# rgl-epfl/differentiable-sdf-rendering

Hardware: AMD Instinct MI355X
Metric: diff-renders/sec (fwd+bwd) 256^3 SDF, 512^2, 12 views (higher is better)
Workload: dtype f32; 1 GPU; no-tex-12-hq sizes: 256^3 SDF, 12 views x 512^2, sdf_silhouette_reparam, spp primal/grad 256/64 (reference semantics, configs.py:16,19); views_total=12, views_this_rank=12, partition=whole views, spp_primal=256, spp_grad=64, schedule=primal pass and gradient sweep on two HIP streams

## Files before the change

### differentiable-sdf-rendering_amd/csrc/dsdf_kernels.hip

```cpp
#include <hip/hip_runtime.h>
#include <stdio.h>
#include <stdlib.h>
#include <string.h>
#include <mutex>
#include <vector>
#include "dsdf_lane.h"

using namespace dsdf;

#if DSDF_XF
namespace dsdf {
__constant__ XfState g_xf_dev;
XfState g_xf_host = {{1.f, 0.f, 0.f, 0.f, 1.f, 0.f, 0.f, 0.f, 1.f}, {0.f, 0.f, 0.f}, {0.f, 0.f, 0.f}, {1.f, 1.f, 1.f}};
}
#endif

#define DSDF_BLOCK 256
#define DSDF_TSTRIDE 68
#define DSDF_TROWS 13
#define DSDF_WAVE_LDS 1104
#ifndef DSDF_PRIMAL_MINWAVES
#define DSDF_PRIMAL_MINWAVES 8
#endif

// ... 770 lines not shown
    uint32_t *count0;
    unsigned char *skip;
    uint32_t *items;
    char *tail;
    size_t tail_bytes;
    float *hit_t;
    char *shq;
    uint32_t shq_cap_sub;
    uint32_t cap, nunits, tail_cap_sub, tail_words, group_views, coef_rows;
    size_t bytes;
};

static Workspace carve(void *base, int W, int H, int spp, int nv, int integrator, bool diff = true) {
    Workspace ws;
    const size_t nch = (size_t)film_channels(integrator), rows = integrator == DSDF_DIRECT ? 27 : 9;
    size_t Wb = W + 2 * DSDF_BORDER, Hb = H + 2 * DSDF_BORDER;
    size_t nunits;
    int tile_w, tile_h;
    pass_shape(W, H, spp, tile_w, tile_h, nunits);
    size_t cap = nunits * 64;
    size_t off = 0;
    char *p = (char *)base;
    ws.block = (float *)(p + off); off += align_up(nv * Wb * Hb * nch * sizeof(float), 256);
    ws.skip = (unsigned char *)(p + off); off += align_up(nv * Wb * Hb, 256);
    ws.items = (uint32_t *)(p + off); off += align_up((DSDF_MAX_GROUPS * DSDF_ITEM_HDR + nv * Wb * Hb) * sizeof(uint32_t), 256);
    ws.block_adj = nullptr; ws.count = nullptr; ws.qlane = nullptr; ws.qrec = nullptr; ws.qcoef = nullptr; ws.coef_rows = 0; ws.count0 = nullptr;
    ws.tail = nullptr; ws.tail_bytes = 0; ws.tail_cap_sub = 0; ws.tail_words = 0; ws.hit_t = nullptr; ws.shq = nullptr; ws.shq_cap_sub = 0;
    ws.group_views = (uint32_t)((nv + DSDF_MAX_GROUPS - 1) / DSDF_MAX_GROUPS);
    if (diff) {
        ws.block_adj = (float *)(p + off); off += align_up(nv * Wb * Hb * nch * sizeof(float), 256);
        ws.count = (uint32_t *)(p + off); off += align_up(nv * nunits * sizeof(uint32_t), 256);
        ws.qlane = (uint32_t *)(p + off); off += align_up(nv * cap * sizeof(uint32_t), 256);
        ws.qrec = (float *)(p + off); off += align_up(nv * cap * rows * sizeof(float), 256);
        if (integrator != DSDF_DIRECT) {
            ws.coef_rows = integrator == DSDF_SILHOUETTE ? 8 : DSDF_COEF_WORDS;
            ws.qcoef = (float *)(p + off); off += align_up(nv * cap * ws.coef_rows * sizeof(float), 256);
            ws.count0 = (uint32_t *)(p + off); off += align_up(nv * nunits * sizeof(uint32_t), 256);
        }
    }
    if (spp % 64 == 0) {
        const size_t handoff = diff ? DSDF_TAIL_HANDOFF : DSDF_PTAIL_HANDOFF;
        ws.tail_words = diff ? DSDF_TAIL_WORDS : DSDF_PTAIL_WORDS;
        ws.tail_cap_sub = (uint32_t)((ws.group_views * Wb * Hb * (size_t)(spp / 64) + DSDF_TAIL_SUBQ - 1) / DSDF_TAIL_SUBQ * handoff);
        ws.tail_bytes = align_up((size_t)DSDF_MAX_GROUPS * DSDF_TAIL_SUBQ * DSDF_TAIL_CNT_STRIDE * sizeof(uint32_t), 256) +
                        (size_t)DSDF_MAX_GROUPS * align_up((size_t)DSDF_TAIL_SUBQ * ws.tail_cap_sub * ws.tail_words * sizeof(float), 256);
        ws.tail = p + off; off += ws.tail_bytes;
    }
// ... 189 lines not shown
    hipLaunchKernelGGL(k_pad_grid, dim3(grid), dim3(256), 0, (hipStream_t)stream, data, rx, ry, rz, padded);
    int rc = check_launch("k_pad_grid");
    if (rc) return rc;
    float *c0 = padded + n;
    for (int l = 0; l < DSDF_COARSE_LEVELS; ++l) {
        int cx, cy, cz;
        coarse_dims(rx, ry, rz, l, cx, cy, cz);
        int nc = cx * cy * cz;
        float *c1 = c0 + nc;
        hipLaunchKernelGGL(k_coarse_reduce<false>, dim3((nc + 63) / 64), dim3(64), 0, (hipStream_t)stream, data, rx, ry, rz, c0, cx, cy, cz,
                           1 << DSDF_COARSE_SHIFT(l));
        hipLaunchKernelGGL(k_coarse_dilate<false>, dim3((nc + 63) / 64), dim3(64), 0, (hipStream_t)stream, c0, c1, cx, cy, cz, 1);
        c0 = c1 + nc;
    }
    {
        int cx, cy, cz;
        hit_dims(rx, ry, rz, cx, cy, cz);
        int nc = cx * cy * cz;
        float *c1 = c0 + nc;
        hipLaunchKernelGGL(k_coarse_reduce<true>, dim3((nc + 255) / 256), dim3(256), 0, (hipStream_t)stream, data, rx, ry, rz, c0, cx, cy, cz,
                           1 << DSDF_HIT_SHIFT);
        hipLaunchKernelGGL(k_coarse_dilate<true>, dim3((nc + 255) / 256), dim3(256), 0, (hipStream_t)stream, c0, c1, cx, cy, cz, DSDF_HIT_RADIUS);
    }
    {
        float *F = fine_buffer(padded, rx, ry, rz), *S = F + (size_t)rx * ry * rz;
        const size_t total = (size_t)rx * ry * rz;
        const dim3 g((unsigned)((total + 255) / 256)), b(256);
        const hipStream_t st = (hipStream_t)stream;
#if DSDF_TLAYOUT
        float *T = padded + tlayout_offset(rx, ry, rz);
        hipLaunchKernelGGL(k_window<false>, g, b, 0, st, data, S, total, rx, (size_t)1, DSDF_FINE_LO, DSDF_FINE_HI);
        hipLaunchKernelGGL(k_window<false>, g, b, 0, st, (const float *)S, T, total, ry, (size_t)rx, DSDF_FINE_LO, DSDF_FINE_HI);
        hipLaunchKernelGGL(k_window<false>, g, b, 0, st, (const float *)T, S, total, rz, (size_t)rx * ry, DSDF_FINE_LO, DSDF_FINE_HI);
#else
        float *T = S;
#endif
        hipLaunchKernelGGL(k_window<true>, g, b, 0, st, data, F, total, rx, (size_t)1, DSDF_FINE_LO, DSDF_FINE_HI);
        hipLaunchKernelGGL(k_window<true>, g, b, 0, st, (const float *)F, T, total, ry, (size_t)rx, DSDF_FINE_LO, DSDF_FINE_HI);
        hipLaunchKernelGGL(k_window<true>, g, b, 0, st, (const float *)T, F, total, rz, (size_t)rx * ry, DSDF_FINE_LO, DSDF_FINE_HI);
    }
    if ((rc = check_launch("k_coarse_reduce/dilate/window"))) return rc;
#if DSDF_TLAYOUT
    {
        const int sx = rx + 2 * DSDF_APRON, sy = ry + 2 * DSDF_APRON, sz = rz + 2 * DSDF_APRON, nxc = (int)tlayout_chunks(rx);
        const size_t nt = (size_t)nxc * sz * sy * 2;
        const int tg = (int)((nt + 255) / 256 < 16384 ? (nt + 255) / 256 : 16384);
// ... 128 lines not shown
    return g_events[g_next_event++ % g_events.size()];
}

static thread_local unsigned long long *g_tail_stats = nullptr;
static thread_local hipEvent_t g_time_ev[2] = {nullptr, nullptr};
static thread_local int g_time_state = 0;

static void timing_mark(int which, hipStream_t st) {
    if (g_time_state != 1 && !(which == 1 && g_time_state == 3)) return;
    if (which == 0) { if (hipEventRecord(g_time_ev[0], st) == hipSuccess) g_time_state = 3; }
    else { if (hipEventRecord(g_time_ev[1], st) == hipSuccess) g_time_state = 2; }
}

struct SkipShare {
    unsigned char *buf = nullptr;
    size_t bytes = 0;
    bool valid = false;
    hipEvent_t ready = nullptr;
    int device = -1;
    const float *padded = nullptr;
    int rx = 0, ry = 0, rz = 0, W = 0, H = 0, nv = 0;
    int hit_proof = 0;
    int fine_empty = 0;
    dsdf_params prm;
    dsdf_camera cams[DSDF_MAX_BATCH];
};
static thread_local SkipShare t_share;

static bool skip_share_matches(const SkipShare &h, const PassCtx &c, const dsdf_camera *cams, int nv) {
    return h.valid && h.padded == c.padded && h.rx == c.rx && h.ry == c.ry && h.rz == c.rz && h.W == c.W && h.H == c.H && h.nv == nv &&
           h.hit_proof <= (int)(c.integrator == DSDF_SILHOUETTE && !(c.flags & DSDF_NO_HIT_PROOF)) &&
           h.fine_empty <= (int)!(c.flags & DSDF_NO_FINE_EMPTY) &&
           memcmp(&h.prm, c.prm, sizeof(dsdf_params)) == 0 && memcmp(h.cams, cams, (size_t)nv * sizeof(dsdf_camera)) == 0;
}

static int pixel_proof(const PassCtx &c, const Workspace &ws, const dsdf_camera *cams, int nv, const ViewBatch &VB,
                       const unsigned char *&skip) {
    int rc;
    hipStream_t st = c.st;
    const size_t npix = c.Wb * c.Hb;
    skip = nullptr;
    float step = 0.f;
    const int level = (c.flags & DSDF_NO_SKIP) ? -1 : skip_level(cams, nv, c.W, c.rx, c.ry, c.rz, step);
    if (level < 0) return DSDF_OK;
    SkipShare &sh = t_share;
    const bool can_share = sh.buf && sh.ready && sh.bytes >= (size_t)nv * npix;
    if (can_share && skip_share_matches(sh, c, cams, nv)) {
        if (hipStreamWaitEvent(st, sh.ready, 0) != hipSuccess) return fail(DSDF_ERR_LAUNCH, "hipStreamWaitEvent(shared skip flags) failed");
        skip = sh.buf;
        return DSDF_OK;
    }
    unsigned char *dst = (can_share && !sh.valid) ? sh.buf : ws.skip;
    const bool want_hit = c.integrator == DSDF_SILHOUETTE && !(c.flags & DSDF_NO_HIT_PROOF) && c.spp >= HIT_PROOF_MIN_SPP;
    const float hstep = want_hit ? hit_step(cams, nv, c.W, c.rx, c.ry, c.rz) : 0.f;
    const float fstep = hit_step_fine(cams, nv, c.W, c.rx, c.ry, c.rz);
    const BoundGrid none = {nullptr, 0, 0, 0, 0, 0.f};
    const BoundGrid fmin = (c.flags & DSDF_NO_FINE_EMPTY) ? none : fine_min_bounds(c.padded, c.rx, c.ry, c.rz);
    const bool fine = fstep > 0.f && (want_hit || fmin.b);
    const int list_g = (fmin.b && (c.diff || dst == sh.buf)) ? 1 : 0;
    uint32_t *und = fine ? ws.items + (size_t)DSDF_MAX_GROUPS * DSDF_ITEM_HDR - DSDF_UNDECIDED_HDR : nullptr;
    if (und && hipMemsetAsync(und, 0, sizeof(uint32_t), st) != hipSuccess) return fail(DSDF_ERR_LAUNCH, "hipMemsetAsync(undecided list) failed");
    const float step0 = level > 0 ? skip_step(cams, nv, c.W, c.rx, c.ry, c.rz, level - 1) : 0.f;
    const dim3 pgrid((unsigned)((npix + 255) / 256), nv), blk(256);
    if ((rc = launch("k_pixel_skip", k_pixel_skip, pgrid, blk, st, device_view(c), min_bounds(c.padded, c.rx, c.ry, c.rz, level > 0 ? level - 1 : 0),
                     min_bounds(c.padded, c.rx, c.ry, c.rz, level), max_bounds(c.padded, c.rx, c.ry, c.rz), c.pp, VB, dst, step0, step, hstep, und, list_g)))
        return rc;
    if (und && (rc = launch("k_pixel_hit_fine", k_pixel_hit_fine, dim3((unsigned)((npix * nv + 255) / 256)), blk, st, device_view(c),
                            fmin, fine_bounds(c.padded, c.rx, c.ry, c.rz), c.pp, VB, dst, und, und + DSDF_UNDECIDED_HDR, fstep, (int)want_hit)))
        return rc;
    if ((rc = launch("k_skip_dilate", k_skip_dilate, pgrid, blk, st, VB, dst))) return rc;
    if (dst == sh.buf) {
        if (hipEventRecord(sh.ready, st) != hipSuccess) return fail(DSDF_ERR_LAUNCH, "hipEventRecord(shared skip flags) failed");
        sh.valid = true; sh.padded = c.padded; sh.rx = c.rx; sh.ry = c.ry; sh.rz = c.rz; sh.W = c.W; sh.H = c.H; sh.nv = nv;
        sh.hit_proof = (int)want_hit;
        sh.fine_empty = (int)(fine && fmin.b);
        sh.prm = *c.prm;
        memcpy(sh.cams, cams, (size_t)nv * sizeof(dsdf_camera));
    }
    skip = dst;
    return DSDF_OK;
}

struct Batch {
    const ViewBatch &VB;
    int nv;
    GridView G;
    ShadeArgs S;
    Queue q;
    float *film;
    const unsigned char *skip;
    unsigned long long *st64;
    bool deep_skip;
    bool env_fill;
};

template <bool DIFF>
static int prefill_film(const PassCtx &c, const Batch &b) {
    int rc;
    const dim3 grid((unsigned)((c.Wb * c.Hb + 255) / 256), b.nv), blk(256);
    if (b.deep_skip && (rc = launch("k_film_ones", k_film_ones, grid, blk, c.st, b.VB, b.skip, b.film, c.row0, c.row1, b.st64))) return rc;
    if (b.env_fill && (rc = launch("k_film_env", k_film_env, grid, blk, c.st, b.VB, b.skip, b.film, c.row0, c.row1,
                                   DIFF ? DSDF_PX_EMPTY_G : (DSDF_PX_EMPTY | DSDF_PX_EMPTY_FINE), b.S.env[0], b.S.env[1], b.S.env[2])))
// ... 448 lines not shown
```

### differentiable-sdf-rendering_amd/csrc/dsdf_proof.h

```cpp
#pragma once
#include "dsdf_math.h"

#define DSDF_PX_EMPTY 1u
#define DSDF_PX_EMPTY_G 2u
#define DSDF_PX_FAR 4u
#define DSDF_PX_FAR_G 8u
#define DSDF_PX_HIT 16u
#define DSDF_PX_DEEP 32u
#define DSDF_PX_ONE 64u
#define DSDF_PX_EMPTY_FINE 128u
#define DSDF_PX_KEEP (DSDF_PX_EMPTY | DSDF_PX_EMPTY_G | DSDF_PX_HIT | DSDF_PX_EMPTY_FINE)

namespace dsdf {

DSDF_HD bool px_primal_empty(unsigned f) { return (f & (DSDF_PX_EMPTY | DSDF_PX_EMPTY_FINE)) != 0u; }
template <bool DIFF> DSDF_HD bool px_skip_trace(unsigned f) { return DIFF ? (f & DSDF_PX_EMPTY_G) != 0u : px_primal_empty(f); }

struct BoundGrid {
    const float *b;
    int cx, cy, cz, shift;
    float off;
};

DSDF_HD float bound_at(const BoundGrid &B, const GridView &G, V3 x) {
// ... 37 lines not shown
    float J = -INFINITY, Jrun = 0.f;
    bool in_run = false;
    for (float tb = t0; tb < t1 + step; tb += 4.f * step) {
        float tc[4], U[4];
#pragma unroll
        for (int k = 0; k < 4; ++k) {
            tc[k] = fminf(tb + (float)k * step, t1);
            U[k] = bound_at(B, G, fma3(tc[k], d, o));
        }
#pragma unroll
        for (int k = 0; k < 4; ++k) {
            if (!(tb + (float)k * step < t1 + step)) break;
            const bool neg = U[k] < 0.f && tc[k] - half >= i0 && tc[k] + half <= i1;
            if (neg) {
                if (!in_run) { in_run = true; Jrun = J; }
                if (tc[k] + half >= Jrun + 1e-4f) return DSDF_PX_HIT;
            } else in_run = false;
            J = fmaxf(J, tc[k] + half + U[k]);
        }
    }
    return 0u;
}

}

static void coarse_dims(int rx, int ry, int rz, int level, int &cx, int &cy, int &cz) {
    const int C = 1 << DSDF_COARSE_SHIFT(level);
    cx = (rx + C - 1) / C; cy = (ry + C - 1) / C; cz = (rz + C - 1) / C;
}
static size_t coarse_cells(int rx, int ry, int rz, int level) {
    int cx, cy, cz;
    coarse_dims(rx, ry, rz, level, cx, cy, cz);
    return (size_t)cx * cy * cz;
}
#define DSDF_HIT_SHIFT 1
#define DSDF_HIT_RADIUS 2
static void hit_dims(int rx, int ry, int rz, int &cx, int &cy, int &cz) {
    const int C = 1 << DSDF_HIT_SHIFT;
    cx = (rx + C - 1) / C; cy = (ry + C - 1) / C; cz = (rz + C - 1) / C;
}
static size_t hit_cells(int rx, int ry, int rz) {
    int cx, cy, cz;
    hit_dims(rx, ry, rz, cx, cy, cz);
    return (size_t)cx * cy * cz;
}

// ... 18 lines not shown
    return step_vox / (float)rmax;
}

static int skip_level(const dsdf_camera *cams, int nv, int W, int rx, int ry, int rz, float &step) {
    for (int level = DSDF_COARSE_LEVELS - 1; level >= 0; --level) {
        step = skip_step(cams, nv, W, rx, ry, rz, level);
        if (step > 0.f) return level;
    }
    step = 0.f;
    return -1;
}

#define DSDF_FINE_LO (-2)
#define DSDF_FINE_HI 3
static float hit_step_fine(const dsdf_camera *cams, int nv, int W, int rx, int ry, int rz) {
    int rmax = rx > ry ? (rx > rz ? rx : rz) : (ry > rz ? ry : rz);
    int rmin = rx < ry ? (rx < rz ? rx : rz) : (ry < rz ? ry : rz);
    const float worst = pixel_spread_voxels(cams, nv, W, rmax);
    if (worst / (float)rmin > 0.5f * DSDF_PROOF_GROW) return 0.f;
    float step_vox = 2.f * (1.f - worst) - 0.02f;
    if (step_vox < 0.25f) return 0.f;
    if (step_vox > 1.f) step_vox = 1.f;
    return step_vox / (float)rmax;
}

static float hit_step(const dsdf_camera *cams, int nv, int W, int rx, int ry, int rz) {
    int rmax = rx > ry ? (rx > rz ? rx : rz) : (ry > rz ? ry : rz);
    int rmin = rx < ry ? (rx < rz ? rx : rz) : (ry < rz ? ry : rz);
    const float worst = pixel_spread_voxels(cams, nv, W, rmax);
    if (worst / (float)rmin > 0.5f * DSDF_PROOF_GROW) return 0.f;
    const float reach = (float)(DSDF_HIT_RADIUS << DSDF_HIT_SHIFT);
    float step_vox = 2.f * (reach - 2.5f - worst);
    if (step_vox < 1.f) return 0.f;
    if (step_vox > 2.f) step_vox = 2.f;
    return step_vox / (float)rmax;
}
```

### differentiable-sdf-rendering_amd/csrc/dsdf_skip.h

```cpp
#pragma once

template <bool MAX>
__global__ void k_coarse_reduce(const float *__restrict__ data, int rx, int ry, int rz, float *__restrict__ c0, int cx, int cy, int cz,
                                int C) {
    int i = blockIdx.x * blockDim.x + threadIdx.x;
    if (i >= cx * cy * cz) return;
    int bx = i % cx, by = (i / cx) % cy, bz = i / (cx * cy);
    float m = MAX ? -INFINITY : INFINITY;
    for (int z = bz * C; z < min(rz, (bz + 1) * C); ++z)
        for (int y = by * C; y < min(ry, (by + 1) * C); ++y)
            for (int x = bx * C; x < min(rx, (bx + 1) * C); ++x) {
                const float v = data[((size_t)z * ry + y) * rx + x];
                m = MAX ? fmaxf(m, v) : fminf(m, v);
            }
    c0[i] = m;
}

template <bool MAX>
__global__ void k_coarse_dilate(const float *__restrict__ c0, float *__restrict__ c, int cx, int cy, int cz, int radius) {
    int i = blockIdx.x * blockDim.x + threadIdx.x;
    if (i >= cx * cy * cz) return;
    int bx = i % cx, by = (i / cx) % cy, bz = i / (cx * cy);
    float m = MAX ? -INFINITY : INFINITY;
    for (int z = max(bz - radius, 0); z <= min(bz + radius, cz - 1); ++z)
        for (int y = max(by - radius, 0); y <= min(by + radius, cy - 1); ++y)
            for (int x = max(bx - radius, 0); x <= min(bx + radius, cx - 1); ++x) {
                const float v = c0[((size_t)z * cy + y) * cx + x];
                m = MAX ? fmaxf(m, v) : fminf(m, v);
            }
    c[i] = m;
}

template <bool MAX>
__global__ void k_window(const float *__restrict__ in, float *__restrict__ out, size_t total, int n, size_t st, int lo, int hi) {
    const size_t i = (size_t)blockIdx.x * blockDim.x + threadIdx.x;
    if (i >= total) return;
    const int a = (int)((i / st) % (size_t)n);
    float m = MAX ? -INFINITY : INFINITY;
    for (int o = lo; o <= hi; ++o) {
        const int b = min(max(a + o, 0), n - 1);
        const float v = in[i + (size_t)(b - a) * st];
        m = MAX ? fmaxf(m, v) : fminf(m, v);
    }
    out[i] = m;
}

#define DSDF_UNDECIDED_HDR 16
__global__ void k_pixel_skip(GridView G, BoundGrid Bmin0, BoundGrid Bmin, BoundGrid Bmax, dsdf_params P, ViewBatch VB,
                             unsigned char *__restrict__ flags, float step0, float step, float hstep, uint32_t *__restrict__ undecided,
                             int list_g) {
    const ViewArgs &A = VB.v[blockIdx.y];
    const int i = blockIdx.x * blockDim.x + threadIdx.x, npix = A.Wb * A.Hb;
    const bool valid = i < npix;
    unsigned f = DSDF_PX_EMPTY;
    if (valid) {
        int py = i / A.Wb, px = i - py * A.Wb;
        CamRay r = camera_ray(A.cam, P, (float)(px - DSDF_BORDER) + 0.5f, (float)(py - DSDF_BORDER) + 0.5f, A.W, A.H);
        V3 d = r.d * rsqf(dot(r.d, r.d));
        if (step0 > 0.f) f = pixel_empty_proof(G, Bmin0, P, r.o, d, step0);
        else f = 0u;
        if (f != (DSDF_PX_EMPTY | DSDF_PX_EMPTY_G) && step > 0.f) f |= pixel_empty_proof(G, Bmin, P, r.o, d, step);
        if (hstep > 0.f && !(f & DSDF_PX_EMPTY)) f |= pixel_hit_proof(G, Bmax, P, r.o, d, hstep);
        flags[(size_t)blockIdx.y * npix + i] = (unsigned char)f;
    }
    if (undecided) {
        const bool open = valid && (!(f & (DSDF_PX_EMPTY | DSDF_PX_HIT)) || (list_g && (f & 3u) == DSDF_PX_EMPTY));
        const uint64_t m = __ballot(open);
        if (m != 0) {
            const int leader = __builtin_ctzll(m);
            uint32_t base = 0;
            if (lane_id() == leader) base = atomicAdd(undecided, (uint32_t)__popcll(m));
            base = (uint32_t)__builtin_amdgcn_readlane((int)base, leader);
            if (open) undecided[DSDF_UNDECIDED_HDR + base + mask_prefix(m)] = (uint32_t)blockIdx.y * (uint32_t)npix + (uint32_t)i;
        }
    }
}

__global__ __launch_bounds__(256) void k_pixel_hit_fine(GridView G, BoundGrid Bmin, BoundGrid B, dsdf_params P, ViewBatch VB,
                                                        unsigned char *__restrict__ flags, const uint32_t *__restrict__ count,
                                                        const uint32_t *__restrict__ list, float step, int hit) {
    const uint32_t i = blockIdx.x * blockDim.x + threadIdx.x;
    if (i >= *count) return;
    const uint32_t e = list[i], npix = (uint32_t)(VB.v[0].Wb * VB.v[0].Hb), view = e / npix, pix = e - view * npix;
    const ViewArgs &A = VB.v[view];
    const int py = (int)(pix / (uint32_t)A.Wb), px = (int)(pix - (uint32_t)py * (uint32_t)A.Wb);
    const CamRay r = camera_ray(A.cam, P, (float)(px - DSDF_BORDER) + 0.5f, (float)(py - DSDF_BORDER) + 0.5f, A.W, A.H);
    const V3 d = r.d * rsqf(dot(r.d, r.d));
    const unsigned f = flags[e];
    unsigned add = 0u;
    if (Bmin.b) {
        const unsigned m = pixel_empty_proof(G, Bmin, P, r.o, d, step);
        add = ((m & DSDF_PX_EMPTY) ? DSDF_PX_EMPTY_FINE : 0u) | (m & DSDF_PX_EMPTY_G);
    }
    if (hit && !add && !(f & DSDF_PX_EMPTY)) add = pixel_hit_proof(G, B, P, r.o, d, step);
    if (add) flags[e] = (unsigned char)(f | add);
}

#define DSDF_FAR_RADIUS 4
__global__ void k_skip_dilate(ViewBatch VB, unsigned char *__restrict__ flags) {
    const ViewArgs &A = VB.v[blockIdx.y];
    int i = blockIdx.x * blockDim.x + threadIdx.x;
    if (i >= A.Wb * A.Hb) return;
    unsigned char *f = flags + (size_t)blockIdx.y * A.Wb * A.Hb;
    int py = i / A.Wb, px = i - py * A.Wb;
    unsigned m = 3u | DSDF_PX_HIT, near = DSDF_PX_HIT;
    for (int y = max(py - DSDF_FAR_RADIUS, 0); y <= min(py + DSDF_FAR_RADIUS, A.Hb - 1); ++y)
        for (int x = max(px - DSDF_FAR_RADIUS, 0); x <= min(px + DSDF_FAR_RADIUS, A.Wb - 1); ++x) {
            const unsigned v = f[y * A.Wb + x];
            m &= v | (px_primal_empty(v) ? DSDF_PX_EMPTY : 0u);
            if (abs(y - py) <= 2 && abs(x - px) <= 2) near &= v;
        }
    f[i] = (unsigned char)((f[i] & DSDF_PX_KEEP) | ((m & 3u) << 2) | ((m & DSDF_PX_HIT) ? DSDF_PX_DEEP : 0u) | (near ? DSDF_PX_ONE : 0u));
}

__global__ void k_film_env(ViewBatch VB, const unsigned char *__restrict__ flags, float *__restrict__ blocks, int row0, int row1,
                           unsigned pass_mask, float er, float eg, float eb) {
    const ViewArgs &A = VB.v[blockIdx.y];
    const int i = blockIdx.x * blockDim.x + threadIdx.x, npix = A.Wb * A.Hb;
    if (i >= npix) return;
    const int py = i / A.Wb, px = i - py * A.Wb;
    if (py < row0 || py >= row1) return;
    const unsigned char *f = flags + (size_t)blockIdx.y * npix;
    bool m = true;
    for (int y = max(py - 2, 0); y <= min(py + 2, A.Hb - 1); ++y)
        for (int x = max(px - 2, 0); x <= min(px + 2, A.Wb - 1); ++x) m = m && (f[y * A.Wb + x] & pass_mask) != 0u;
    if (!m) return;
    float *b = blocks + ((size_t)blockIdx.y * npix + i) * 4;
    atomicAdd(b, er); atomicAdd(b + 1, eg); atomicAdd(b + 2, eb); atomicAdd(b + 3, 1.f);
}

__global__ void k_film_ones(ViewBatch VB, const unsigned char *__restrict__ flags, float *__restrict__ blocks, int row0, int row1,
                            unsigned long long *stats) {
    const ViewArgs &A = VB.v[blockIdx.y];
    const int i = blockIdx.x * blockDim.x + threadIdx.x, npix = A.Wb * A.Hb;
    const int py = i < npix ? i / A.Wb : -1;
// ... 21 lines not shown
#endif
    return G;
}
static BoundGrid min_bounds(const float *padded, int rx, int ry, int rz, int level) {
    const float *c = padded + padded_floats(rx, ry, rz);
    for (int l = 0; l < level; ++l) c += 2 * coarse_cells(rx, ry, rz, l);
    BoundGrid B;
    coarse_dims(rx, ry, rz, level, B.cx, B.cy, B.cz);
    B.shift = DSDF_COARSE_SHIFT(level);
    B.off = 0.f;
    B.b = c + coarse_cells(rx, ry, rz, level);
    return B;
}
static BoundGrid max_bounds(const float *padded, int rx, int ry, int rz) {
    const float *c = padded + padded_floats(rx, ry, rz);
    for (int l = 0; l < DSDF_COARSE_LEVELS; ++l) c += 2 * coarse_cells(rx, ry, rz, l);
    BoundGrid B;
    hit_dims(rx, ry, rz, B.cx, B.cy, B.cz);
    B.shift = DSDF_HIT_SHIFT;
    B.off = 0.f;
    B.b = c + hit_cells(rx, ry, rz);
    return B;
}
static float *fine_buffer(const float *padded, int rx, int ry, int rz) {
    const float *c = padded + padded_floats(rx, ry, rz);
    for (int l = 0; l < DSDF_COARSE_LEVELS; ++l) c += 2 * coarse_cells(rx, ry, rz, l);
    return const_cast<float *>(c) + 2 * hit_cells(rx, ry, rz);
}
static size_t tlayout_offset(int rx, int ry, int rz) {
    size_t n = padded_floats(rx, ry, rz);
    for (int l = 0; l < DSDF_COARSE_LEVELS; ++l) n += 2 * coarse_cells(rx, ry, rz, l);
    n += 2 * hit_cells(rx, ry, rz) + 2 * (size_t)rx * ry * rz;
    return (n + 3) & ~(size_t)3;
}
static BoundGrid fine_bounds(const float *padded, int rx, int ry, int rz) {
    BoundGrid B;
    B.cx = rx; B.cy = ry; B.cz = rz; B.shift = 0; B.off = 0.5f;
    B.b = fine_buffer(padded, rx, ry, rz);
    return B;
}
static BoundGrid fine_min_bounds(const float *padded, int rx, int ry, int rz) {
    BoundGrid B = fine_bounds(padded, rx, ry, rz);
#if DSDF_TLAYOUT
    B.b += (size_t)rx * ry * rz;
#else
    B.b = nullptr;
// ... 4 lines not shown
```

### differentiable-sdf-rendering_amd/python/dsdf/_lib.py

```python
import ctypes as C
import os

_HERE = os.path.dirname(os.path.abspath(__file__))
LIB_PATH = os.environ.get('DSDF_LIB_PATH') or os.path.normpath(os.path.join(_HERE, '..', '..', 'lib', 'libdsdf.so'))

DSDF_SILHOUETTE = 0
DSDF_SIMPLE_SHADING = 1
DSDF_DIRECT = 2
DSDF_REPARAM = 1
DSDF_NO_SKIP = 2
DSDF_NO_HIT_PROOF = 4
DSDF_NO_FINE_EMPTY = 8


class DsdfCamera(C.Structure):
    _fields_ = [('origin', C.c_float * 3), ('left', C.c_float * 3), ('up', C.c_float * 3),
                ('dir', C.c_float * 3), ('tan_half_fov', C.c_float), ('pad', C.c_float * 3)]


class DsdfParams(C.Structure):
    _fields_ = [('trace_eps', C.c_float), ('extra_thresh', C.c_float), ('sil_weight_offset', C.c_float),
                ('sil_weight_epsilon', C.c_float), ('bbox_delta', C.c_float), ('edge_eps', C.c_float),
                ('clamping_thresh', C.c_float), ('near_clip', C.c_float), ('far_clip', C.c_float),
                ('sdf_p', C.c_float * 3), ('weight_strategy', C.c_int), ('refine_steps', C.c_int),
                ('light_dir', C.c_float * 3), ('normalize_warp_field', C.c_int), ('max_reparam_depth', C.c_int)]


class DsdfShading(C.Structure):
    _fields_ = [('albedo', C.c_void_p), ('ax', C.c_int), ('ay', C.c_int), ('az', C.c_int),
                ('env_radiance', C.c_float * 3), ('hide_emitters', C.c_int), ('emitter_samples', C.c_void_p),
                ('grad_albedo', C.c_void_p), ('use_mis', C.c_int), ('variant', C.c_int), ('bsdf_samples', C.c_void_p),
                ('bsdf', C.c_int), ('roughness', C.c_void_p), ('rax', C.c_int), ('ray', C.c_int), ('raz', C.c_int),
                ('grad_roughness', C.c_void_p), ('bsdf_lobe_samples', C.c_void_p)]


# ... 137 lines not shown
```

### differentiable-sdf-rendering_amd/python/dsdf/parallel.py

```python
import math

import torch


def view_shard(n_views, rank, world):
    if world < 1 or not (0 <= rank < world):
        raise ValueError(f"bad rank/world {rank}/{world}")
    base, extra = divmod(n_views, world)
    start = rank * base + min(rank, extra)
    return list(range(start, start + base + (1 if rank < extra else 0)))


def strided_view_shard(indices, rank, world):
    return list(indices)[rank::world]


def work_partition(n_views, film_rows, world):
    if world < 1 or n_views < 1:
        raise ValueError("bad n_views / world")
    tiles = world // math.gcd(n_views, world)
    edges = [round(k * film_rows / tiles) for k in range(tiles + 1)]
    units = [(v, edges[k], edges[k + 1]) for v in range(n_views) for k in range(tiles)]
    return [units[r::world] for r in range(world)]

# ... 14 lines not shown
    for v in sorted(range(n_views), key=lambda i: (-vc[i], i)):
        g = min((g for g in range(G) if len(groups[g]) < per_group), key=lambda g: (sums[g], g))
        groups[g].append(v); sums[g] += vc[v]
    out = []
    for g in range(G):
        views = sorted(groups[g])
        h = cost[views].sum(0) + 1e-12 * max(vc.sum(), 1.0) / rows
        c = np.concatenate([[0.0], np.cumsum(h)])
        edges = [0]
        for k in range(1, tiles):
            e = int(np.searchsorted(c, c[-1] * k / tiles))
            if e > 0 and abs(c[e - 1] - c[-1] * k / tiles) <= abs(c[e] - c[-1] * k / tiles):
                e -= 1
            e = max(edges[-1] + 1, min(e, rows - (tiles - k)))
            edges.append(e)
        edges.append(rows)
        for k in range(tiles):
            out.append([(v, edges[k], edges[k + 1]) for v in views])
    return out


def row_costs(flags, n_views, Wb, Hb, spp, spp_grad, silhouette=True):
    import torch
    f = flags[:n_views * Wb * Hb].view(n_views, Hb, Wb)
    empty, empty_g, far, far_g, hit, deep = ((f & b) != 0 for b in (1, 2, 4, 8, 16, 32))
    listed_p = ~far & ~(deep if silhouette else torch.zeros_like(deep))
    proven_p = listed_p & (empty | (hit if silhouette else torch.zeros_like(hit)))
    traced_p = listed_p & ~proven_p
    listed_g = ~far_g
    traced_g = listed_g & ~empty_g
    cp, cg = spp / 64.0, spp_grad / 64.0
    c = cp * (5600.0 * traced_p.sum(2, dtype=torch.float64) + 500.0 * proven_p.sum(2, dtype=torch.float64)) + \
        cg * (15000.0 * traced_g.sum(2, dtype=torch.float64) + 500.0 * (listed_g & ~traced_g).sum(2, dtype=torch.float64))
    return c


def rank_windows(units):
    out = {}
    for v, r0, r1 in units:
        out.setdefault((r0, r1), []).append(v)
    return sorted(out.items())


def all_reduce_sum(t, group=None):
    import torch.distributed as dist
    if dist.is_available() and dist.is_initialized() and dist.get_world_size(group) > 1:
        dist.all_reduce(t, op=dist.ReduceOp.SUM, group=group)
    return t
# ... 154 lines not shown
        self.seeds, self.seeds_grad = list(seeds), list(seeds_grad)

    def empty_film(self, n):
        return self.r.new_film(n, self.W, self.H, self.integrator, self.grid.device)

    def film(self, views, rows):
        f = self.empty_film(len(views))
        return self.r.render_film(self.grid, [self.sensors[v] for v in views], self.spp, f, rows,
                                  seeds=[self.seeds[v] for v in views], integrator=self.integrator, **self.kw_film)

    def develop(self, film):
        return self.r.develop(film, self.W, self.H, self.integrator)

    def begin_group(self, views):
        import torch
        dev = self.grid.device
        n = len(views) * (self.W + 4) * (self.H + 4)
        self._group_views = list(views)
        bufs = self.__dict__.setdefault('_flag_bufs', [])
        gi = getattr(self, '_group_i', 0)
        self._group_i = gi + 1
        while len(bufs) <= gi:
            bufs.append(None)
        if bufs[gi] is None or bufs[gi].numel() < n:
            bufs[gi] = torch.empty(n, dtype=torch.uint8, device=dev)
        self._flags = bufs[gi]
        self._share_lib = self.r.share_proof_open(self.grid, self.kw.get('shading'), self._flags)

    def end_group(self):
        self.r.share_proof_close(self.grid, self._share_lib)
        self._flag_views = getattr(self, '_group_views', None)

    def row_costs(self):
        views = getattr(self, '_flag_views', None)
        if not views or getattr(self, '_flags', None) is None:
            return [], None
        from .renderer import DSDF_SILHOUETTE
        sil = self.integrator in (DSDF_SILHOUETTE, 'sdf_silhouette_reparam')
        return list(views), row_costs(self._flags, len(views), self.W + 4, self.H + 4, self.spp, self.spp_grad, sil)

    def begin_sweeps(self):
        import torch
        self._next_ws = 0
        self._group_i = 0
        if self._side is not None:
            self._side.wait_stream(torch.cuda.current_stream(self.grid.device))
            self._in_sweeps = True

    def end_sweeps(self):
# ... 141 lines not shown
```

### differentiable-sdf-rendering_amd/python/dsdf/renderer.py

```python
import contextlib
import ctypes as C

import os

import torch

from . import _lib
from ._lib import (DSDF_DIRECT, DSDF_NO_FINE_EMPTY, DSDF_NO_HIT_PROOF, DSDF_NO_SKIP, DSDF_REPARAM, DSDF_SILHOUETTE, DSDF_SIMPLE_SHADING, DsdfCamera,
                   DsdfShading)

INTEGRATORS = {'sdf_silhouette_reparam': DSDF_SILHOUETTE, 'sdf_simple_shading_reparam': DSDF_SIMPLE_SHADING,
               'sdf_direct_reparam': DSDF_DIRECT,
               DSDF_SILHOUETTE: DSDF_SILHOUETTE, DSDF_SIMPLE_SHADING: DSDF_SIMPLE_SHADING, DSDF_DIRECT: DSDF_DIRECT}

STAT_NAMES = ('lanes', 'bbox_lanes', 'steps', 'hits', 'refine_steps', 'warp_active', 'queue_len', 'wave_steps',
              'tail_steps', 'tail_wave_steps', 'tail_rays')
STAT_SLOTS = 16

_workspaces = {}


def _proof_flags(empty_space_skip):
    if empty_space_skip == 'empty-only':
        return DSDF_NO_HIT_PROOF
    if empty_space_skip == 'coarse-empty':
        return DSDF_NO_FINE_EMPTY
    return 0 if empty_space_skip else DSDF_NO_SKIP

MAX_VIEWS_PER_LAUNCH = 16


def _stream():
    return C.c_void_p(torch.cuda.current_stream().cuda_stream)


def _ptr(t):
    return C.c_void_p(t.data_ptr()) if t is not None else C.c_void_p(0)


def _floats(a):
    return (C.c_float * len(a))(*[float(v) for v in a])


def _as_list(sensors):
    return list(sensors) if isinstance(sensors, (list, tuple)) else [sensors]


def _require_dev(t, name, dtype=torch.float32):
    if not isinstance(t, torch.Tensor) or not t.is_cuda:
# ... 548 lines not shown
        yield
    finally:
        share_proof_close(grid, lib)


def _lease_sweep_workspace(dev):
    ent = _sweep_workspaces.get(dev)
    if ent is None or ent['leased']:
        return None, None
    ent['leased'] = True
    return ent['ws'], ent


def step_begin(grid, sensors, spp, spp_grad, seeds, seeds_grad, integrator=DSDF_SILHOUETTE, reparam=True, shading=None,
               grad_albedo=None, empty_space_skip=True):
    sensors = _as_list(sensors)
    W, H = sensors[0].film_size()
    dev = grid.device
    main = torch.cuda.current_stream(dev)
    side = _side_streams.get(dev)
    if side is None:
        side = _side_streams[dev] = torch.cuda.Stream(dev, priority=-1)
    side.wait_stream(main)
    nflag = len(sensors) * (W + 4) * (H + 4)
    flags = _skip_buffers.get(dev)
    if flags is None or flags.numel() < nflag:
        flags = _skip_buffers[dev] = torch.empty(nflag, dtype=torch.uint8, device=dev)
    share = os.environ.get('DSDF_SHARE_SKIP', '1') != '0'
    with torch.cuda.device(dev), (shared_proof(grid, shading, flags) if share else contextlib.nullcontext()):
        ws, lease = _lease_sweep_workspace(dev)
        with torch.cuda.stream(side):
            sweep = GradSweep(grid, sensors, spp_grad, (0, H + 4), seeds=seeds_grad, integrator=integrator, reparam=reparam,
                              shading=shading, grad_albedo=grad_albedo, workspace=ws, empty_space_skip=empty_space_skip)
            if sweep.ws is not None and sweep.ws is not ws:
                if lease is not None:
                    lease['leased'] = False
                lease = _sweep_workspaces[dev] = {'ws': sweep.ws, 'leased': True}
            film_g = sweep.sweep(new_film(len(sensors), W, H, integrator, dev))
        img = render_forward(grid, sensors, spp, seeds=seeds, integrator=integrator, reparam=reparam, shading=shading,
                             empty_space_skip=empty_space_skip)
    return img, StepHandle(sweep, film_g, main, side, lease)


def step_finish(handle, grad_image, grad_grid, grad_p=None):
    if handle.done:
        sw = handle.sweep
        sw.make_private()
# ... 283 lines not shown
```

### include/dsdf.h

```cpp
#ifndef DSDF_H
#define DSDF_H

#include <stddef.h>
#include <stdint.h>

#ifdef __cplusplus
extern "C" {
#endif

#define DSDF_VERSION 308
#define DSDF_STAT_SLOTS 16

enum dsdf_status {
    DSDF_OK = 0,
    DSDF_ERR_INVALID_ARG = -1,
    DSDF_ERR_WORKSPACE = -2,
    DSDF_ERR_LAUNCH = -3,
    DSDF_ERR_NO_DEVICE = -4
};

enum dsdf_integrator {
    DSDF_SILHOUETTE = 0,
    DSDF_SIMPLE_SHADING = 1,
    DSDF_DIRECT = 2
};

enum dsdf_flags {
    DSDF_REPARAM = 1,
    DSDF_NO_SKIP = 2,
    DSDF_NO_HIT_PROOF = 4,
    DSDF_NO_FINE_EMPTY = 8
};

typedef struct dsdf_camera {
    float origin[3];
    float left[3];
    float up[3];
    float dir[3];
    float tan_half_fov;
    float pad[3];
} dsdf_camera;

typedef struct dsdf_params {
    float trace_eps;
    float extra_thresh;
    float sil_weight_offset;
    float sil_weight_epsilon;
    float bbox_delta;
    float edge_eps;
    float clamping_thresh;
    float near_clip;
    float far_clip;
    float sdf_p[3];
    int   weight_strategy;
// ... 153 lines not shown
```

Baseline: 30.79 renders/s.

## Tighten per-pixel empty/hit proofs with a Lipschitz value bound from grid tap differences

Adds a kernel that computes the maximum neighbouring-voxel difference along each axis of the SDF grid. The fine proof pass uses this as a gradient bound, evaluating the actual SDF value with a Lipschitz margin to tighten the min/max bounds along each ray. This lets more pixels be proven empty or hit and skipped in the primal and gradient passes. The proof results go into a second flag plane, so the skip buffers double in size and the dilate and row-cost logic read that plane. The cost is an extra grid reduction and extra SDF evaluations during proof building.

```diff
diff --git a/differentiable-sdf-rendering_amd/csrc/dsdf_kernels.hip b/differentiable-sdf-rendering_amd/csrc/dsdf_kernels.hip
--- a/differentiable-sdf-rendering_amd/csrc/dsdf_kernels.hip
+++ b/differentiable-sdf-rendering_amd/csrc/dsdf_kernels.hip
@@ -816,7 +816,7 @@
     size_t off = 0;
     char *p = (char *)base;
     ws.block = (float *)(p + off); off += align_up(nv * Wb * Hb * nch * sizeof(float), 256);
-    ws.skip = (unsigned char *)(p + off); off += align_up(nv * Wb * Hb, 256);
+    ws.skip = (unsigned char *)(p + off); off += align_up(2 * nv * Wb * Hb, 256);
     ws.items = (uint32_t *)(p + off); off += align_up((DSDF_MAX_GROUPS * DSDF_ITEM_HDR + nv * Wb * Hb) * sizeof(uint32_t), 256);
     ws.block_adj = nullptr; ws.count = nullptr; ws.qlane = nullptr; ws.qrec = nullptr; ws.qcoef = nullptr; ws.coef_rows = 0; ws.count0 = nullptr;
     ws.tail = nullptr; ws.tail_bytes = 0; ws.tail_cap_sub = 0; ws.tail_words = 0; ws.hit_t = nullptr; ws.shq = nullptr; ws.shq_cap_sub = 0;
@@ -1052,6 +1052,11 @@
                            1 << DSDF_HIT_SHIFT);
         hipLaunchKernelGGL(k_coarse_dilate<true>, dim3((nc + 255) / 256), dim3(256), 0, (hipStream_t)stream, c0, c1, cx, cy, cz, DSDF_HIT_RADIUS);
     }
+    if (float *D = grad_bound(padded, rx, ry, rz)) {
+        if (hipMemsetAsync(D, 0, 3 * sizeof(float), (hipStream_t)stream) != hipSuccess) return fail(DSDF_ERR_LAUNCH, "hipMemsetAsync(gradient bound) failed");
+        const unsigned g = (unsigned)((size_t)ry * rz < 4096 ? (size_t)ry * rz : 4096);
+        hipLaunchKernelGGL(k_tap_diff_max, dim3(g), dim3(256), 0, (hipStream_t)stream, data, rx, ry, rz, (int *)D);
+    }
     {
         float *F = fine_buffer(padded, rx, ry, rz), *S = F + (size_t)rx * ry * rz;
         const size_t total = (size_t)rx * ry * rz;
@@ -1226,6 +1231,7 @@
     int rx = 0, ry = 0, rz = 0, W = 0, H = 0, nv = 0;
     int hit_proof = 0;
     int fine_empty = 0;
+    int value_bound = 0;
     dsdf_params prm;
     dsdf_camera cams[DSDF_MAX_BATCH];
 };
@@ -1235,6 +1241,7 @@
     return h.valid && h.padded == c.padded && h.rx == c.rx && h.ry == c.ry && h.rz == c.rz && h.W == c.W && h.H == c.H && h.nv == nv &&
            h.hit_proof <= (int)(c.integrator == DSDF_SILHOUETTE && !(c.flags & DSDF_NO_HIT_PROOF)) &&
            h.fine_empty <= (int)!(c.flags & DSDF_NO_FINE_EMPTY) &&
+           h.value_bound <= (int)!(c.flags & (DSDF_NO_FINE_EMPTY | DSDF_NO_VALUE_BOUND)) &&
            memcmp(&h.prm, c.prm, sizeof(dsdf_params)) == 0 && memcmp(h.cams, cams, (size_t)nv * sizeof(dsdf_camera)) == 0;
 }
 
@@ -1251,7 +1258,7 @@
     const bool can_share = sh.buf && sh.ready && sh.bytes >= (size_t)nv * npix;
     if (can_share && skip_share_matches(sh, c, cams, nv)) {
         if (hipStreamWaitEvent(st, sh.ready, 0) != hipSuccess) return fail(DSDF_ERR_LAUNCH, "hipStreamWaitEvent(shared skip flags) failed");
-        skip = sh.buf;
+        skip = sh.value_bound ? sh.buf + (size_t)nv * npix : sh.buf;
         return DSDF_OK;
     }
     unsigned char *dst = (can_share && !sh.valid) ? sh.buf : ws.skip;
@@ -1262,26 +1269,33 @@
     const BoundGrid fmin = (c.flags & DSDF_NO_FINE_EMPTY) ? none : fine_min_bounds(c.padded, c.rx, c.ry, c.rz);
     const bool fine = fstep > 0.f && (want_hit || fmin.b);
     const int list_g = (fmin.b && (c.diff || dst == sh.buf)) ? 1 : 0;
+    ValueBound vb = {nullptr, 0.f};
+    if (fine && fmin.b && !(c.flags & DSDF_NO_VALUE_BOUND) && (dst != sh.buf || sh.bytes >= 2 * (size_t)nv * npix)) {
+        vb.D = grad_bound(c.padded, c.rx, c.ry, c.rz);
+        vb.r = value_bound_reach(cams, nv, c.W, c.rx, c.ry, c.rz, fstep);
+    }
+    unsigned char *plane = vb.D ? dst + (size_t)nv * npix : nullptr;
     uint32_t *und = fine ? ws.items + (size_t)DSDF_MAX_GROUPS * DSDF_ITEM_HDR - DSDF_UNDECIDED_HDR : nullptr;
     if (und && hipMemsetAsync(und, 0, sizeof(uint32_t), st) != hipSuccess) return fail(DSDF_ERR_LAUNCH, "hipMemsetAsync(undecided list) failed");
     const float step0 = level > 0 ? skip_step(cams, nv, c.W, c.rx, c.ry, c.rz, level - 1) : 0.f;
     const dim3 pgrid((unsigned)((npix + 255) / 256), nv), blk(256);
     if ((rc = launch("k_pixel_skip", k_pixel_skip, pgrid, blk, st, device_view(c), min_bounds(c.padded, c.rx, c.ry, c.rz, level > 0 ? level - 1 : 0),
-                     min_bounds(c.padded, c.rx, c.ry, c.rz, level), max_bounds(c.padded, c.rx, c.ry, c.rz), c.pp, VB, dst, step0, step, hstep, und, list_g)))
+                     min_bounds(c.padded, c.rx, c.ry, c.rz, level), max_bounds(c.padded, c.rx, c.ry, c.rz), c.pp, VB, dst, step0, step, hstep, und, list_g, plane)))
         return rc;
     if (und && (rc = launch("k_pixel_hit_fine", k_pixel_hit_fine, dim3((unsigned)((npix * nv + 255) / 256)), blk, st, device_view(c),
-                            fmin, fine_bounds(c.padded, c.rx, c.ry, c.rz), c.pp, VB, dst, und, und + DSDF_UNDECIDED_HDR, fstep, (int)want_hit)))
+                            fmin, fine_bounds(c.padded, c.rx, c.ry, c.rz), vb, c.pp, VB, dst, plane, und, und + DSDF_UNDECIDED_HDR, fstep, (int)want_hit)))
         return rc;
-    if ((rc = launch("k_skip_dilate", k_skip_dilate, pgrid, blk, st, VB, dst))) return rc;
+    if ((rc = launch("k_skip_dilate", k_skip_dilate, pgrid, blk, st, VB, dst, plane))) return rc;
     if (dst == sh.buf) {
         if (hipEventRecord(sh.ready, st) != hipSuccess) return fail(DSDF_ERR_LAUNCH, "hipEventRecord(shared skip flags) failed");
         sh.valid = true; sh.padded = c.padded; sh.rx = c.rx; sh.ry = c.ry; sh.rz = c.rz; sh.W = c.W; sh.H = c.H; sh.nv = nv;
         sh.hit_proof = (int)want_hit;
         sh.fine_empty = (int)(fine && fmin.b);
+        sh.value_bound = (int)(plane != nullptr);
         sh.prm = *c.prm;
         memcpy(sh.cams, cams, (size_t)nv * sizeof(dsdf_camera));
     }
-    skip = dst;
+    skip = plane ? plane : dst;
     return DSDF_OK;
 }
 
diff --git a/differentiable-sdf-rendering_amd/csrc/dsdf_proof.h b/differentiable-sdf-rendering_amd/csrc/dsdf_proof.h
--- a/differentiable-sdf-rendering_amd/csrc/dsdf_proof.h
+++ b/differentiable-sdf-rendering_amd/csrc/dsdf_proof.h
@@ -83,6 +83,93 @@
     return 0u;
 }
 
+struct ValueBound {
+    const float *D;
+    float r;
+};
+struct ValueMargin { float L, tap; };
+DSDF_HD ValueMargin value_margin(const ValueBound &vb) {
+    const float dn = sqrtf(vb.D[0] * vb.D[0] + vb.D[1] * vb.D[1] + vb.D[2] * vb.D[2]);
+    ValueMargin m;
+    m.L = vb.r * dn * (1.f + 1e-5f);
+    m.tap = 3.f * (vb.D[0] + vb.D[1] + vb.D[2]);
+    return m;
+}
+
+struct HitRun {
+    float J, Jrun;
+    bool in_run, done;
+};
+DSDF_HD void hit_run_step(HitRun &s, float U, float tc, float half, bool inside) {
+    if (s.done) return;
+    if (U < 0.f && inside) {
+        if (!s.in_run) { s.in_run = true; s.Jrun = s.J; }
+        if (tc + half >= s.Jrun + 1e-4f) { s.done = true; return; }
+    } else s.in_run = false;
+    s.J = fmaxf(s.J, tc + half + U);
+}
+
+DSDF_HD unsigned pixel_fine_proofs(const GridView &G, const BoundGrid &Bmin, const BoundGrid &Bmax, const ValueBound &vb, const dsdf_params &P,
+                                   V3 o, V3 d, float step, bool want_hit) {
+    BoxHit b = bbox_ray_intersect(-P.bbox_delta - DSDF_PROOF_GROW, 1.f + P.bbox_delta + DSDF_PROOF_GROW, o, d);
+    if (!(b.hit && b.maxt > 0.f)) return 0u;
+    BoxHit in = bbox_ray_intersect(-P.bbox_delta + DSDF_PROOF_GROW, 1.f + P.bbox_delta - DSDF_PROOF_GROW, o, d);
+    want_hit = want_hit && P.trace_eps > 0.f && in.hit && in.maxt > 0.f;
+    const bool want_empty = Bmin.b != nullptr, third = want_empty && vb.D != nullptr;
+    const float t0 = fmaxf(b.mint, 0.f), t1 = b.maxt, half = 0.5f * step;
+    const float i0 = fmaxf(in.mint, 0.f), i1 = in.maxt;
+    const float thr_p = 2.f * P.trace_eps * fmaxf(t1, 1.f) + 1e-5f;
+    const float thr_g = (P.weight_strategy == 6 ? P.edge_eps * (t1 + 0.1f) : P.edge_eps) * 1.05f + 1e-4f;
+    const float thr_hi = fmaxf(thr_p, thr_g);
+    ValueMargin mg = {0.f, 0.f};
+    if (third) mg = value_margin(vb);
+    float m2 = INFINITY, m3 = INFINITY;
+    HitRun h2 = {-INFINITY, 0.f, false, false}, h3 = h2;
+    bool e_alive = want_empty;
+    for (float tb = t0; tb < t1 + step && (e_alive || (want_hit && !h2.done)); tb += 4.f * step) {
+        float tc[4], lo[4], hi[4], lo3[4], hi3[4];
+        const bool v_alive = third && (e_alive || (want_hit && !h3.done));
+        const bool fetch_lo = e_alive || v_alive;
+#pragma unroll
+        for (int k = 0; k < 4; ++k) {
+            const bool live = tb + (float)k * step < t1 + step;
+            tc[k] = fminf(tb + (float)k * step, t1);
+            const V3 x = fma3(tc[k], d, o);
+            lo3[k] = lo[k] = fetch_lo && live ? bound_at(Bmin, G, x) : INFINITY;
+            hi3[k] = hi[k] = want_hit ? bound_at(Bmax, G, x) : INFINITY;
+            const bool need_e = e_alive && lo[k] <= (m3 > thr_hi ? thr_hi : thr_p);
+            const bool need_h = want_hit && !h3.done && hi[k] >= 0.f && lo[k] < -mg.L;
+            if (v_alive && live && (need_e || need_h)) {
+                const float v = eval_value(G, x), m = mg.L + 4e-6f * (fabsf(v) + mg.tap);
+                lo3[k] = fmaxf(lo[k], v - m);
+                hi3[k] = fminf(hi[k], v + m);
+            }
+        }
+        m2 = fminf(m2, fminf(fminf(lo[0], lo[1]), fminf(lo[2], lo[3])));
+        m3 = fminf(m3, fminf(fminf(lo3[0], lo3[1]), fminf(lo3[2], lo3[3])));
+        if (want_hit) {
+#pragma unroll
+            for (int k = 0; k < 4; ++k) {
+                if (!(tb + (float)k * step < t1 + step)) break;
+                const bool inside = tc[k] - half >= i0 && tc[k] + half <= i1;
+                hit_run_step(h2, hi[k], tc[k], half, inside);
+                hit_run_step(h3, hi3[k], tc[k], half, inside);
+            }
+        }
+        e_alive = want_empty && m3 > thr_p;
+    }
+    unsigned f2 = 0u, f3 = 0u;
+    if (want_empty) {
+        if (m2 > thr_p) f2 |= DSDF_PX_EMPTY;
+        if (m2 > thr_hi) f2 |= DSDF_PX_EMPTY_G;
+        if (m3 > thr_p) f3 |= DSDF_PX_EMPTY;
+        if (m3 > thr_hi) f3 |= DSDF_PX_EMPTY_G;
+    }
+    if (!f2 && want_hit && h2.done) f2 = DSDF_PX_HIT;
+    if (!f3 && want_hit && h3.done) f3 = DSDF_PX_HIT;
+    return third ? (f2 | (f3 << 8)) : f2;
+}
+
 }
 
 static void coarse_dims(int rx, int ry, int rz, int level, int &cx, int &cy, int &cz) {
@@ -147,6 +234,11 @@
     if (step_vox < 0.25f) return 0.f;
     if (step_vox > 1.f) step_vox = 1.f;
     return step_vox / (float)rmax;
+}
+
+static float value_bound_reach(const dsdf_camera *cams, int nv, int W, int rx, int ry, int rz, float fstep) {
+    int rmax = rx > ry ? (rx > rz ? rx : rz) : (ry > rz ? ry : rz);
+    return pixel_spread_voxels(cams, nv, W, rmax) + 0.5f * fstep * (float)rmax + 0.01f;
 }
 
 static float hit_step(const dsdf_camera *cams, int nv, int W, int rx, int ry, int rz) {
diff --git a/differentiable-sdf-rendering_amd/csrc/dsdf_skip.h b/differentiable-sdf-rendering_amd/csrc/dsdf_skip.h
--- a/differentiable-sdf-rendering_amd/csrc/dsdf_skip.h
+++ b/differentiable-sdf-rendering_amd/csrc/dsdf_skip.h
@@ -45,10 +45,32 @@
     out[i] = m;
 }
 
+__global__ __launch_bounds__(256) void k_tap_diff_max(const float *__restrict__ data, int rx, int ry, int rz, int *__restrict__ D) {
+    float mx = 0.f, my = 0.f, mz = 0.f;
+    for (int row = blockIdx.x; row < ry * rz; row += gridDim.x) {
+        const int y = row % ry, z = row / ry;
+        const float *r = data + (size_t)row * rx;
+        for (int x = threadIdx.x; x < rx; x += blockDim.x) {
+            const float v = r[x];
+            if (x + 1 < rx) mx = fmaxf(mx, fabsf(r[x + 1] - v));
+            if (y + 1 < ry) my = fmaxf(my, fabsf(r[x + (size_t)rx] - v));
+            if (z + 1 < rz) mz = fmaxf(mz, fabsf(r[x + (size_t)rx * ry] - v));
+        }
+    }
+    __shared__ int part[4][3];
+    const int ix = wave_max_i32(__float_as_int(mx)), iy = wave_max_i32(__float_as_int(my)), iz = wave_max_i32(__float_as_int(mz));
+    if (lane_id() == 0) { part[threadIdx.x >> 6][0] = ix; part[threadIdx.x >> 6][1] = iy; part[threadIdx.x >> 6][2] = iz; }
+    __syncthreads();
+    if (threadIdx.x < 3) {
+        const int m = max(max(part[0][threadIdx.x], part[1][threadIdx.x]), max(part[2][threadIdx.x], part[3][threadIdx.x]));
+        if (m > __atomic_load_n(D + threadIdx.x, __ATOMIC_RELAXED)) atomicMax(D + threadIdx.x, m);
+    }
+}
+
 #define DSDF_UNDECIDED_HDR 16
 __global__ void k_pixel_skip(GridView G, BoundGrid Bmin0, BoundGrid Bmin, BoundGrid Bmax, dsdf_params P, ViewBatch VB,
                              unsigned char *__restrict__ flags, float step0, float step, float hstep, uint32_t *__restrict__ undecided,
-                             int list_g) {
+                             int list_g, unsigned char *__restrict__ plane) {
     const ViewArgs &A = VB.v[blockIdx.y];
     const int i = blockIdx.x * blockDim.x + threadIdx.x, npix = A.Wb * A.Hb;
     const bool valid = i < npix;
@@ -62,6 +84,7 @@
         if (f != (DSDF_PX_EMPTY | DSDF_PX_EMPTY_G) && step > 0.f) f |= pixel_empty_proof(G, Bmin, P, r.o, d, step);
         if (hstep > 0.f && !(f & DSDF_PX_EMPTY)) f |= pixel_hit_proof(G, Bmax, P, r.o, d, hstep);
         flags[(size_t)blockIdx.y * npix + i] = (unsigned char)f;
+        if (plane) plane[(size_t)blockIdx.y * npix + i] = 0;
     }
     if (undecided) {
         const bool open = valid && (!(f & (DSDF_PX_EMPTY | DSDF_PX_HIT)) || (list_g && (f & 3u) == DSDF_PX_EMPTY));
@@ -76,9 +99,10 @@
     }
 }
 
-__global__ __launch_bounds__(256) void k_pixel_hit_fine(GridView G, BoundGrid Bmin, BoundGrid B, dsdf_params P, ViewBatch VB,
-                                                        unsigned char *__restrict__ flags, const uint32_t *__restrict__ count,
-                                                        const uint32_t *__restrict__ list, float step, int hit) {
+__global__ __launch_bounds__(256) void k_pixel_hit_fine(GridView G, BoundGrid Bmin, BoundGrid B, ValueBound vb, dsdf_params P, ViewBatch VB,
+                                                        unsigned char *__restrict__ flags, unsigned char *__restrict__ plane,
+                                                        const uint32_t *__restrict__ count, const uint32_t *__restrict__ list, float step,
+                                                        int hit) {
     const uint32_t i = blockIdx.x * blockDim.x + threadIdx.x;
     if (i >= *count) return;
     const uint32_t e = list[i], npix = (uint32_t)(VB.v[0].Wb * VB.v[0].Hb), view = e / npix, pix = e - view * npix;
@@ -87,30 +111,37 @@
     const CamRay r = camera_ray(A.cam, P, (float)(px - DSDF_BORDER) + 0.5f, (float)(py - DSDF_BORDER) + 0.5f, A.W, A.H);
     const V3 d = r.d * rsqf(dot(r.d, r.d));
     const unsigned f = flags[e];
-    unsigned add = 0u;
-    if (Bmin.b) {
-        const unsigned m = pixel_empty_proof(G, Bmin, P, r.o, d, step);
-        add = ((m & DSDF_PX_EMPTY) ? DSDF_PX_EMPTY_FINE : 0u) | (m & DSDF_PX_EMPTY_G);
-    }
-    if (hit && !add && !(f & DSDF_PX_EMPTY)) add = pixel_hit_proof(G, B, P, r.o, d, step);
+    const unsigned m = pixel_fine_proofs(G, Bmin, B, vb, P, r.o, d, step, hit && !(f & DSDF_PX_EMPTY));
+    const unsigned m2 = m & 0xffu, m3 = m >> 8;
+    const unsigned add = ((m2 & DSDF_PX_EMPTY) ? DSDF_PX_EMPTY_FINE : 0u) | (m2 & (DSDF_PX_EMPTY_G | DSDF_PX_HIT));
     if (add) flags[e] = (unsigned char)(f | add);
+    const unsigned add3 = ((m3 & DSDF_PX_EMPTY) ? DSDF_PX_EMPTY_FINE : 0u) | (m3 & (DSDF_PX_EMPTY_G | DSDF_PX_HIT));
+    if (plane && add3) plane[e] = (unsigned char)add3;
 }
 
 #define DSDF_FAR_RADIUS 4
-__global__ void k_skip_dilate(ViewBatch VB, unsigned char *__restrict__ flags) {
+__global__ void k_skip_dilate(ViewBatch VB, unsigned char *__restrict__ flags, unsigned char *__restrict__ plane) {
     const ViewArgs &A = VB.v[blockIdx.y];
     int i = blockIdx.x * blockDim.x + threadIdx.x;
     if (i >= A.Wb * A.Hb) return;
     unsigned char *f = flags + (size_t)blockIdx.y * A.Wb * A.Hb;
+    unsigned char *p = plane ? plane + (size_t)blockIdx.y * A.Wb * A.Hb : nullptr;
     int py = i / A.Wb, px = i - py * A.Wb;
-    unsigned m = 3u | DSDF_PX_HIT, near = DSDF_PX_HIT;
+    unsigned m = 3u | DSDF_PX_HIT, near = DSDF_PX_HIT, m3 = m, near3 = near;
     for (int y = max(py - DSDF_FAR_RADIUS, 0); y <= min(py + DSDF_FAR_RADIUS, A.Hb - 1); ++y)
         for (int x = max(px - DSDF_FAR_RADIUS, 0); x <= min(px + DSDF_FAR_RADIUS, A.Wb - 1); ++x) {
             const unsigned v = f[y * A.Wb + x];
             m &= v | (px_primal_empty(v) ? DSDF_PX_EMPTY : 0u);
             if (abs(y - py) <= 2 && abs(x - px) <= 2) near &= v;
+            if (p) {
+                const unsigned w = v | (p[y * A.Wb + x] & DSDF_PX_KEEP);
+                m3 &= w | (px_primal_empty(w) ? DSDF_PX_EMPTY : 0u);
+                if (abs(y - py) <= 2 && abs(x - px) <= 2) near3 &= w;
+            }
         }
-    f[i] = (unsigned char)((f[i] & DSDF_PX_KEEP) | ((m & 3u) << 2) | ((m & DSDF_PX_HIT) ? DSDF_PX_DEEP : 0u) | (near ? DSDF_PX_ONE : 0u));
+    const unsigned own = f[i];
+    f[i] = (unsigned char)((own & DSDF_PX_KEEP) | ((m & 3u) << 2) | ((m & DSDF_PX_HIT) ? DSDF_PX_DEEP : 0u) | (near ? DSDF_PX_ONE : 0u));
+    if (p) p[i] = (unsigned char)(((own | p[i]) & DSDF_PX_KEEP) | ((m3 & 3u) << 2) | ((m3 & DSDF_PX_HIT) ? DSDF_PX_DEEP : 0u) | (near3 ? DSDF_PX_ONE : 0u));
 }
 
 __global__ void k_film_env(ViewBatch VB, const unsigned char *__restrict__ flags, float *__restrict__ blocks, int row0, int row1,
@@ -178,6 +209,12 @@
     B.b = c + hit_cells(rx, ry, rz);
     return B;
 }
+static float *grad_bound(const float *padded, int rx, int ry, int rz) {
+    if (hit_cells(rx, ry, rz) < 3) return nullptr;
+    const float *c = padded + padded_floats(rx, ry, rz);
+    for (int l = 0; l < DSDF_COARSE_LEVELS; ++l) c += 2 * coarse_cells(rx, ry, rz, l);
+    return const_cast<float *>(c);
+}
 static float *fine_buffer(const float *padded, int rx, int ry, int rz) {
     const float *c = padded + padded_floats(rx, ry, rz);
     for (int l = 0; l < DSDF_COARSE_LEVELS; ++l) c += 2 * coarse_cells(rx, ry, rz, l);
diff --git a/differentiable-sdf-rendering_amd/python/dsdf/_lib.py b/differentiable-sdf-rendering_amd/python/dsdf/_lib.py
--- a/differentiable-sdf-rendering_amd/python/dsdf/_lib.py
+++ b/differentiable-sdf-rendering_amd/python/dsdf/_lib.py
@@ -11,6 +11,7 @@
 DSDF_NO_SKIP = 2
 DSDF_NO_HIT_PROOF = 4
 DSDF_NO_FINE_EMPTY = 8
+DSDF_NO_VALUE_BOUND = 16
 
 
 class DsdfCamera(C.Structure):
diff --git a/differentiable-sdf-rendering_amd/python/dsdf/parallel.py b/differentiable-sdf-rendering_amd/python/dsdf/parallel.py
--- a/differentiable-sdf-rendering_amd/python/dsdf/parallel.py
+++ b/differentiable-sdf-rendering_amd/python/dsdf/parallel.py
@@ -60,8 +60,12 @@
 
 def row_costs(flags, n_views, Wb, Hb, spp, spp_grad, silhouette=True):
     import torch
-    f = flags[:n_views * Wb * Hb].view(n_views, Hb, Wb)
-    empty, empty_g, far, far_g, hit, deep = ((f & b) != 0 for b in (1, 2, 4, 8, 16, 32))
+    n = n_views * Wb * Hb
+    f = flags[:n].view(n_views, Hb, Wb)
+    if flags.numel() >= 2 * n:
+        p = flags[n:2 * n].view(n_views, Hb, Wb)
+        f = torch.where(p[0, 0, 0] != 255, p, f)
+    empty, empty_g, far, far_g, hit, deep = ((f & b) != 0 for b in (1 | 128, 2, 4, 8, 16, 32))
     listed_p = ~far & ~(deep if silhouette else torch.zeros_like(deep))
     proven_p = listed_p & (empty | (hit if silhouette else torch.zeros_like(hit)))
     traced_p = listed_p & ~proven_p
@@ -262,9 +266,12 @@
         self._group_i = gi + 1
         while len(bufs) <= gi:
             bufs.append(None)
-        if bufs[gi] is None or bufs[gi].numel() < n:
-            bufs[gi] = torch.empty(n, dtype=torch.uint8, device=dev)
+        if bufs[gi] is None or bufs[gi].numel() < 2 * n:
+            bufs[gi] = torch.empty(2 * n, dtype=torch.uint8, device=dev)
         self._flags = bufs[gi]
+        import contextlib
+        with (torch.cuda.stream(self._side) if (self._side is not None and self._in_sweeps) else contextlib.nullcontext()):
+            self._flags[n:2 * n].fill_(255)
         self._share_lib = self.r.share_proof_open(self.grid, self.kw.get('shading'), self._flags)
 
     def end_group(self):
diff --git a/differentiable-sdf-rendering_amd/python/dsdf/renderer.py b/differentiable-sdf-rendering_amd/python/dsdf/renderer.py
--- a/differentiable-sdf-rendering_amd/python/dsdf/renderer.py
+++ b/differentiable-sdf-rendering_amd/python/dsdf/renderer.py
@@ -6,7 +6,7 @@
 import torch
 
 from . import _lib
-from ._lib import (DSDF_DIRECT, DSDF_NO_FINE_EMPTY, DSDF_NO_HIT_PROOF, DSDF_NO_SKIP, DSDF_REPARAM, DSDF_SILHOUETTE, DSDF_SIMPLE_SHADING, DsdfCamera,
+from ._lib import (DSDF_DIRECT, DSDF_NO_FINE_EMPTY, DSDF_NO_HIT_PROOF, DSDF_NO_VALUE_BOUND, DSDF_NO_SKIP, DSDF_REPARAM, DSDF_SILHOUETTE, DSDF_SIMPLE_SHADING, DsdfCamera,
                    DsdfShading)
 
 INTEGRATORS = {'sdf_silhouette_reparam': DSDF_SILHOUETTE, 'sdf_simple_shading_reparam': DSDF_SIMPLE_SHADING,
@@ -25,6 +25,8 @@
         return DSDF_NO_HIT_PROOF
     if empty_space_skip == 'coarse-empty':
         return DSDF_NO_FINE_EMPTY
+    if empty_space_skip == 'window-empty':
+        return DSDF_NO_VALUE_BOUND
     return 0 if empty_space_skip else DSDF_NO_SKIP
 
 MAX_VIEWS_PER_LAUNCH = 16
@@ -619,7 +621,7 @@
     if side is None:
         side = _side_streams[dev] = torch.cuda.Stream(dev, priority=-1)
     side.wait_stream(main)
-    nflag = len(sensors) * (W + 4) * (H + 4)
+    nflag = 2 * len(sensors) * (W + 4) * (H + 4)
     flags = _skip_buffers.get(dev)
     if flags is None or flags.numel() < nflag:
         flags = _skip_buffers[dev] = torch.empty(nflag, dtype=torch.uint8, device=dev)
diff --git a/include/dsdf.h b/include/dsdf.h
--- a/include/dsdf.h
+++ b/include/dsdf.h
@@ -29,7 +29,8 @@
     DSDF_REPARAM = 1,
     DSDF_NO_SKIP = 2,
     DSDF_NO_HIT_PROOF = 4,
-    DSDF_NO_FINE_EMPTY = 8
+    DSDF_NO_FINE_EMPTY = 8,
+    DSDF_NO_VALUE_BOUND = 16
 };
 
 typedef struct dsdf_camera {
```

After: 32.62 renders/s (median of 6 runs). 6.0% higher.
